# rafaelgmv/Distributed-Autonomous-Exploration-and-Mapping

Measured on AMD Instinct MI355X. Metric: beam-cell updates/sec + frontier-extract ms on 16384² grid, higher is better.
Workload: dtype int32/u32 ray math + fp32 log-odds (fp64 endpoints)

## Files before the change

distributed-autonomous-exploration-and-mapping_amd/csrc/dm_api.cpp:

```cpp
#include <math.h>
#include <stdarg.h>
#include <stdio.h>
#include <string.h>

#include <algorithm>
#include <new>
#include <string>
#include <vector>

#include "dm_internal.h"

#include <stdlib.h>

hipError_t dm_sync_all(dm_grid* g) {
  for (hipStream_t s : {g->stream, g->fe_stream, g->pass_stream, g->big_stream}) {
    if (!s) continue;
    const hipError_t e = hipStreamSynchronize(s);
    if (e != hipSuccess) return e;
  }
  g->p_pending = false;
  for (auto& f : g->fw) f.busy_pending = false;
  return hipSuccess;
}

// ... 452 lines not shown
  for (auto& w : g->iw) {
    if ((rc = dev_alloc(&w.tile_count, g->NT, "tile counts"))) return fail(rc);
    if ((rc = dev_alloc(&w.tile_cur, g->NT, "tile bin cursors"))) return fail(rc);
    if ((rc = dev_alloc(&w.cnt, CNT_N, "integrate counters"))) return fail(rc);
    if ((rc = dev_alloc(&w.sh, kShards * kShardWords, "integrate shard counters"))) return fail(rc);
    DM_HIP(hipMemset(w.cnt, 0, sizeof(unsigned long long) * CNT_N));
    DM_HIP(hipMemset(w.sh, 0, sizeof(unsigned long long) * kShards * kShardWords));
  }
  if ((rc = dev_alloc(&g->tile_free, g->NT, "tile free counts"))) return fail(rc);
  if ((rc = dev_alloc(&g->fmask, g->NT * DM_TILE * 16, "tile free / unknown bit rows"))) return fail(rc);
  if ((rc = dev_alloc(&g->fedge, g->NT * 4, "tile unknown edge words"))) return fail(rc);
  if ((rc = dev_alloc(&g->tile_seen, g->NT, "tile seen flags"))) return fail(rc);
  if (const char* sp = getenv("DM_SPARSE_PIECES")) g->sparse_pieces = std::max(0, atoi(sp));
  const char* fm = getenv("DM_FMASK");
  g->fmask_mode = fm && !strcmp(fm, "on") ? 1 : (fm && !strcmp(fm, "off") ? 2 : 0);
  const char* fk = getenv("DM_FRONTIER_KERNEL");
  g->frontier_kernel = fk && !strcmp(fk, "wave") ? 1 : (fk && !strcmp(fk, "wg") ? 2 : 0);
  if (const char* sm = getenv("DM_SORT_MIN")) g->sort_min = std::max<int64_t>(0, atoll(sm));
  g->fault_gate = dm_env_on("DM_FAULT_GATE");
  if (const char* pr = getenv("DM_PLAN_MAX_ROUNDS")) g->plan_max_rounds = std::max<int64_t>(0, atoll(pr));
  for (auto& f : g->fw) {
    e = hipEventCreateWithFlags(&f.ev_split, hipEventDisableTiming | hipEventDisableSystemFence);
    if (e != hipSuccess) return fail(dm_hip_check(e, "hipEventCreate"));
    if ((rc = dev_alloc(&f.cnt, CNT_N, "frontier counters"))) return fail(rc);
    DM_HIP(hipMemset(f.cnt, 0, sizeof(unsigned long long) * CNT_N));
    if ((rc = dev_alloc(&f.fsh, kShards * kShardWords, "frontier shard counters"))) return fail(rc);
    DM_HIP(hipMemset(f.fsh, 0, sizeof(unsigned long long) * kShards * kShardWords));
    if ((rc = dev_alloc(&f.big_tiles, g->NT, "frontier big tiles"))) return fail(rc);
    if ((rc = dev_alloc(&f.fbits, g->NT * DM_TILE, "frontier bit rows"))) return fail(rc);
    if ((rc = dev_alloc(&f.edge_slot, 2 * g->W, "edge slots"))) return fail(rc);
// ... 77 lines not shown
    if (ev) (void)hipEventDestroy(ev);
  for (auto& r : g->rb) {
    if (r.ev) (void)hipEventDestroy(r.ev);
    if (r.out_clu) (void)hipFree(r.out_clu - kRbRecords);
    if (r.h_out) (void)hipHostFree(r.h_out - kRbHostRecords);
    dev_free(r.m_out);
  }
  if (g->fe_stream) (void)hipStreamDestroy(g->fe_stream);
  if (g->pass_stream) (void)hipStreamDestroy(g->pass_stream);
  if (g->big_stream) (void)hipStreamDestroy(g->big_stream);
  for (auto& f : g->fw) {
    if (f.ev_split) (void)hipEventDestroy(f.ev_split);
    dev_free(f.cnt); dev_free(f.fsh); dev_free(f.big_tiles); dev_free(f.fbits);
    dev_free(f.edge_slot); dev_free(f.slot_parent);
  }
  dev_free(g->fl_n); dev_free(g->bits_flag);
  for (int i = 0; i < 2; ++i) { dev_free(g->flist[i]); dev_free(g->flist_n[i]); }
  for (int b = 0; b < 2; ++b) { dev_free(g->goal_k[b]); dev_free(g->goal_i[b]); }
  dev_free(g->goal_io); dev_free(g->goal_idx);
  dev_free(g->plan_cost); dev_free(g->plan_trav); dev_free(g->plan_travs); dev_free(g->plan_list[0]);
  dev_free(g->plan_list[1]); dev_free(g->plan_stamp); dev_free(g->plan_len); dev_free(g->plan_stat);
  dev_free(g->plan_src); dev_free(g->plan_qxy); dev_free(g->plan_qcost); dev_free(g->plan_qcell);
  dev_free(g->plan_path);
  if (g->h_plan) (void)hipHostFree(g->h_plan);
  dev_free(g->match_V); dev_free(g->match_kern); dev_free(g->match_tiles); dev_free(g->match_pose4);
  dev_free(g->match_trig); dev_free(g->match_ranges); dev_free(g->match_q); dev_free(g->match_vol);
  dev_free(g->match_out);
  dev_free(g->gain_xy); dev_free(g->gain_cell); dev_free(g->gain_out); dev_free(g->gain_skip);
  dev_free(g->gain_memo_cell); dev_free(g->gain_memo_gain);
  for (auto& w : g->iw) {
    dev_free(w.pieces); dev_free(w.hitems); dev_free(w.litems); dev_free(w.heavy_list); dev_free(w.slabs);
// ... 164 lines not shown
  const unsigned long long* fs = g->h_sh + kShards * kShardWords;
  const unsigned long long* ic = g->h_cnt + CNT_N;
  const uint64_t items = ic[CNT_ITEMS] + ic[CNT_LITEMS] + ic[CNT_SITEMS];
  const uint64_t pieces = ic[CNT_SEGS];
  const uint64_t v[kNStats] = {dm_shard_sum(g->h_sh, SH_U),  dm_shard_sum(g->h_sh, SH_T),
                               dm_shard_sum(g->h_sh, SH_TH), pieces,
                               ic[CNT_ACTIVE],               items,
                               ic[CNT_HEAVY],                g->h_cnt[CNT_FL0],
                               dm_shard_sum(fs, SH_SLOT),    g->h_cnt[CNT_CLUSTERS],
                               ic[CNT_SITEMS]};
  for (int32_t i = 0; i < cap && i < kNStats; ++i) out[i] = v[i];
  if (n_out) *n_out = kNStats;
  return DM_OK;
}

int dm_get_state(dm_grid* g, int8_t* out) {
  if (g && g->sh) return (out ? dm_sh_get_state(g, out) : dm_set_error(DM_ERR_INVALID_ARG, "out is NULL"));
  int rc = check_grid(g);
  if (rc || (rc = use_device(g))) return rc;
  if (!out) return dm_set_error(DM_ERR_INVALID_ARG, "out is NULL");
  DM_HIP(hipMemcpyAsync(out, g->state, (size_t)(g->W * g->R), hipMemcpyDeviceToHost, g->stream));
  DM_HIP(hipStreamSynchronize(g->stream));
  return DM_OK;
}

int dm_get_logodds(dm_grid* g, float* out) {
  if (g && g->sh) return (out ? dm_sh_get_logodds(g, out) : dm_set_error(DM_ERR_INVALID_ARG, "out is NULL"));
  int rc = check_grid(g);
  if (rc || (rc = use_device(g))) return rc;
  if (!out) return dm_set_error(DM_ERR_INVALID_ARG, "out is NULL");
// ... 85 lines not shown

int dm_frontiers_export_device(dm_grid* g, void* d_export, int64_t rec_cap) {
  if (int rc0 = not_on_sharded(g, "dm_frontiers_export_device")) return rc0;
  int rc = check_grid(g);
  if (rc || (rc = use_device(g))) return rc;
  if (!d_export || rec_cap < 0) return dm_set_error(DM_ERR_INVALID_ARG, "d_export is NULL or rec_cap < 0");
  if (g->p.min_frontier_size > 1)
    return dm_set_error(DM_ERR_INVALID_ARG,
                        "export needs a band handle with min_frontier_size <= 1 (the size filter "
                        "applies to merged clusters)");
  dm_select_slot(g, g->rb_count < dm_grid::kRbSlots ? (g->rb_head + g->rb_count) % dm_grid::kRbSlots
                                                    : dm_grid::kRbSync);
  hipStream_t es = g->stream;
  if ((rc = dm_enqueue_frontiers(g, false, false, g->overlap, &es))) return rc;
  if ((rc = dm_launch_export(g, es, d_export, rec_cap))) return rc;
  if (es != g->stream) {
    dm_grid::FrWs& f = g->fw[g->fparity];
    DM_HIP(hipEventRecord(f.ev_split, es));
    f.busy = f.ev_split;
    f.busy_pending = true;
    f.busy_pass = g->fr_pass;
    g->p_tail = f.ev_split;
    g->p_pending = true;
    g->p_tail_pass = g->fr_pass;
  } else {
    DM_HIP(dm_mark_ws_free(g));
  }
  g->frontier_valid = true;
  return DM_OK;
}
// ... 1097 lines not shown
```

distributed-autonomous-exploration-and-mapping_amd/csrc/dm_frontier.hip:

```cpp
#include "dm_internal.h"
#include "dm_uf.h"
#include "dm_phase.h"

#include <string.h>

#include <algorithm>

DM_PH_DECL(frontier)
DM_PH_DECL(ftile)

namespace {

constexpr int kFT = 256;
#ifndef DM_FT_OCC
#define DM_FT_OCC 7
#endif
constexpr int kMaxRoots = 1024;

struct FGeom {
  int32_t W, R, row0, TX, TY;
  int32_t has_before, has_after;
  int32_t pad_ = 0;
  int64_t NT;
  int32_t want_mask, want_labels;
// ... 18 lines not shown
__device__ inline void lds_unite(int32_t* par, int32_t a, int32_t b) {
  volatile int32_t* vp = par;
  for (int it = 0; it < 8192; ++it) {
    a = lds_find(vp, a);
    b = lds_find(vp, b);
    if (a == b) return;
    if (a < b) { const int32_t t = a; a = b; b = t; }
    const int32_t old = atomicMin(&par[a], b);
    if (old == a) return;
    a = old;
  }
}

constexpr int kMaxRuns = 2048;

__device__ inline uint64_t upto_mask(int p) {
  return p >= 63 ? ~0ull : ((2ull << p) - 1ull);
}

__device__ inline uint64_t run_starts(uint64_t F) { return F & ~(F << 1); }

__device__ inline int run_end(uint64_t F, int s0) {
  const uint64_t rest = ~(F >> s0);
  return rest ? s0 + __ffsll((unsigned long long)rest) - 2 : 63;
}

__device__ inline int run_of(const int32_t* rbase, const uint64_t* rowF, int y, int p) {
  return rbase[y] + __popcll(run_starts(rowF[y]) & upto_mask(p)) - 1;
}

__device__ inline int root_rank(const uint64_t* s_root, const int32_t* pre, int r) {
  return pre[r >> 6] + __popcll(s_root[r >> 6] & ((1ull << (r & 63)) - 1ull));
}

template <bool EDGE>
__global__ __launch_bounds__(kFT, DM_FT_OCC) void k_frontier_tile_big(
    FGeom g, const uint64_t* __restrict__ fbits, const int32_t* __restrict__ bflag,
    const int32_t* __restrict__ ftiles, const unsigned long long* __restrict__ list_n,
    int32_t* border, unsigned long long* rel,
    long long* __restrict__ slot_label, int32_t* slot_parent,
    long long* __restrict__ slot_own, long long* __restrict__ slot_acc,
    uint8_t* __restrict__ mask, int32_t* __restrict__ cell_slot, int32_t* __restrict__ edge_slot,
    unsigned long long* cnt, unsigned long long* fsh, int count_stats) {
  const unsigned long long stamp = cnt[CNT_STAMP];
  __shared__ uint64_t s_F[DM_TS];
  __shared__ int32_t s_rbase[DM_TS + 1];
  __shared__ int32_t r_par[kMaxRuns];
  __shared__ uint8_t r_s[kMaxRuns], r_y[kMaxRuns];
  __shared__ uint64_t s_root[kMaxRuns / 64];
  __shared__ int32_t s_rootpre[kMaxRuns / 64];
  __shared__ uint32_t szx[kMaxRoots], ssy[kMaxRoots];
  __shared__ int32_t nroots;
  __shared__ long long sbase;
  const int tid = threadIdx.x, lane = __lane_id();
  const int64_t nft = (int64_t)*list_n;
  const int64_t G = gridDim.x;
  __shared__ uint64_t s_todo;
  DM_PH_INIT();
  for (int64_t kb = blockIdx.x; kb < nft; kb += bflag ? 64 * G : G) {
  uint64_t todo = 1ull;
  if (bflag) {
    if (tid < 64) {
      const int64_t q = kb + (int64_t)tid * G;
      const uint64_t m = __ballot(q < nft && bflag[q] != 0);
      if (tid == 0) s_todo = m;
    }
    __syncthreads();
    todo = s_todo;
    __syncthreads();
  }
  while (todo) {
    const int64_t jj = bflag ? kb + (int64_t)(__ffsll((unsigned long long)todo) - 1) * G : kb;
    todo &= todo - 1;
    const int32_t tile = ftiles[jj];
    const uint64_t F = tid < DM_TS ? fbits[jj * DM_TS + tid] : 0ull;
    const int64_t j = tile;
    DM_PH_COUNT(dm_phase_acc_frontier, 16, 1);
    const int32_t tx0 = (tile % g.TX) * DM_TS;
    const int32_t ty0 = (tile / g.TX) * DM_TS;
    DM_PH(dm_phase_acc_frontier, 0);
    int any = 0;
    if (tid < DM_TS) {
      const int y = tid;
      const uint64_t st = run_starts(F);
      s_F[y] = F;
      any = F != 0ull;
      const int c = __popcll(st);
      int incl = c;
      for (int d = 1; d < 64; d <<= 1) {
        const int v = __shfl_up(incl, d);
        if (lane >= d) incl += v;
      }
      s_rbase[y] = incl - c;
      if (y == 63) s_rbase[DM_TS] = incl;
    }
    any = __syncthreads_or(any);
    DM_PH(dm_phase_acc_frontier, 1);
    if (!any) {
      __syncthreads();
      DM_PH(dm_phase_acc_frontier, 8);
      continue;
    }
    {
      const int y = tid >> 2, q = tid & 3;
      const uint64_t st_all = run_starts(s_F[y]);
      const uint64_t below = q ? upto_mask(16 * q - 1) : 0ull;
      uint64_t st = st_all & upto_mask(16 * q + 15) & ~below;
      int r = s_rbase[y] + __popcll(st_all & below);
      while (st) {
        const int s0 = __ffsll((unsigned long long)st) - 1;
        r_s[r] = (uint8_t)s0;
        r_y[r] = (uint8_t)y;
        r_par[r] = r;
        ++r;
        st &= st - 1;
      }
    }
    for (int r = tid; r < kMaxRoots; r += kFT) { szx[r] = 0; ssy[r] = 0; }
    __syncthreads();
    const int nruns = s_rbase[DM_TS];
    if (count_stats && tid == 0) {
      atomicAdd(&fsh[(blockIdx.x % kShards) * kShardWords + SH_RUNS], (unsigned long long)nruns);
      atomicAdd(&fsh[(blockIdx.x % kShards) * kShardWords + SH_FTF], 1ull);
    }
    DM_PH(dm_phase_acc_frontier, 2);
    DM_PH_COUNT(dm_phase_acc_frontier, 17, nruns);
    DM_PH_COUNT(dm_phase_acc_frontier, 18, 1);
    for (int r = tid; r < nruns; r += kFT) {
      const int y = r_y[r];
      if (y == 0) continue;
      const int s0 = r_s[r], e0 = run_end(s_F[y], s0);
      const int lo = s0 > 0 ? s0 - 1 : 0;
      const int hi = e0 < 63 ? e0 + 1 : 63;
      const uint64_t M = upto_mask(hi) & ~(lo > 0 ? upto_mask(lo - 1) : 0ull);
      uint64_t P = s_F[y - 1] & M;
      while (P) {
        const int p = __ffsll((unsigned long long)P) - 1;
        lds_unite(r_par, r, run_of(s_rbase, s_F, y - 1, p));
// ... 17 lines not shown
    __syncthreads();
    DM_PH(dm_phase_acc_frontier, 4);
    if (tid < 64) {
      const int nw = (nruns + 63) >> 6;
      const int c = tid < nw ? __popcll(s_root[tid]) : 0;
      int incl = c;
      for (int d = 1; d < 64; d <<= 1) {
        const int v = __shfl_up(incl, d);
        if (lane >= d) incl += v;
      }
      if (tid < nw) s_rootpre[tid] = incl - c;
      if (tid == 63) nroots = incl;
    }
    __syncthreads();
    DM_PH(dm_phase_acc_frontier, 5);
    if (tid == 0)
      sbase = (long long)atomicAdd(&fsh[(blockIdx.x % kShards) * kShardWords + SH_SLOT],
                                   (unsigned long long)nroots);
    for (int r = tid; r < nruns; r += kFT) {
      const int c = root_rank(s_root, s_rootpre, r_par[r]);
      const int y = r_y[r];
      const uint32_t s0 = r_s[r], e0 = (uint32_t)run_end(s_F[y], (int)s0), len = e0 - s0 + 1;
      atomicAdd(&szx[c], (len << 18) + (s0 + e0) * len / 2);
      atomicAdd(&ssy[c], (uint32_t)y * len);
    }
    __syncthreads();
    DM_PH(dm_phase_acc_frontier, 6);
    const long long base = sbase;
    const long long sh0 = (long long)(blockIdx.x % kShards) * g.slot_per;
    for (int r = tid; r < nruns; r += kFT) {
      if (r_par[r] != r) continue;
      const int c = root_rank(s_root, s_rootpre, r);
      if (base + c >= g.slot_per) { atomicOr(&cnt[CNT_OVERFLOW], kOvSlots); continue; }
      const long long slot = sh0 + base + c;
      const long long gy = (long long)g.row0 + ty0 + r_y[r];
      const long long gx = (long long)tx0 + r_s[r];
      const uint32_t zx = szx[c];
      const long long sz = zx >> 18;
      slot_label[slot] = gy * g.W + gx;
      const long long sx = sz * tx0 + (zx & 0x3FFFFu);
      const long long sy = sz * ((long long)g.row0 + ty0) + ssy[c];
      slot_own[3 * slot + 0] = sz; slot_own[3 * slot + 1] = sx; slot_own[3 * slot + 2] = sy;
      slot_acc[3 * slot + 0] = sz; slot_acc[3 * slot + 1] = sx; slot_acc[3 * slot + 2] = sy;
    }
    {
      const int side = tid >> 6, pos = lane;
      const int y = side == 0 ? 0 : side == 1 ? 63 : pos;
      const int x = side == 0 || side == 1 ? pos : side == 2 ? 0 : 63;
      int32_t sl = -1;
      if ((s_F[y] >> x) & 1ull) {
        const long long v = base + root_rank(s_root, s_rootpre, r_par[run_of(s_rbase, s_F, y, x)]);
        sl = v < g.slot_per ? (int32_t)(sh0 + v) : -1;
      }
      const uint64_t fb = __ballot(sl >= 0);
      if constexpr (EDGE) {
      if (fb) {
        border[j * 256 + tid] = sl;
        if (lane == 0) rel[4 * g.NT + 4 * j + side] = stamp;
      }
      } else {
      if (fb) {
        __hip_atomic_store(&border[j * 256 + tid], sl, __ATOMIC_RELAXED, __HIP_MEMORY_SCOPE_AGENT);
        asm volatile("s_waitcnt vmcnt(0)" ::: "memory");
        const int32_t tx = tile % g.TX, ty = tile / g.TX;
        const bool up = ty > 0, down = ty + 1 < g.TY, left = tx > 0, right = tx + 1 < g.TX;
        int64_t e = -1;
// ... 44 lines not shown
        }
        {
          const int32_t c0 = __shfl(sl, 0), c63 = __shfl(sl, 63);
          if (second && lane != 0) {
            const int32_t me = lane == 1 ? c0 : c63;
            const int nrow = side == 0 ? 1 : 0;
            const int ncol = lane == 1 ? 63 : 0;
            const int32_t b = __hip_atomic_load(&border[(int64_t)nb * 256 + nrow * 64 + ncol], __ATOMIC_RELAXED,
                                                __HIP_MEMORY_SCOPE_AGENT);
            if (me >= 0 && b >= 0) dm_uf_unite_idx(slot_parent, me, b, &cnt[CNT_OVERFLOW], kOvUnionFind);
          }
        }
      }
      }
    }
    const bool dense = g.want_mask || g.want_labels;
    if (dense || ty0 == 0 || ty0 + DM_TS >= g.R) {
      for (int c = tid; c < DM_TS * DM_TS; c += kFT) {
        const int y = c >> 6, x = c & 63;
        const int32_t gy = ty0 + y, gx = tx0 + x;
        if (gx >= g.W || gy >= g.R) continue;
        const bool edge = gy == 0 || gy == g.R - 1;
        if (!dense && !edge) continue;
        const bool f = (s_F[y] >> x) & 1ull;
        long long sl = -1;
        if (f) {
          sl = base + root_rank(s_root, s_rootpre, r_par[run_of(s_rbase, s_F, y, x)]);
          sl = sl < g.slot_per ? sh0 + sl : -1;
        }
        const int64_t gi = (int64_t)gy * g.W + gx;
        if (g.want_mask) mask[gi] = f;
        if (g.want_labels) cell_slot[gi] = (int32_t)sl;
        if (f) {
          if (gy == 0) edge_slot[gx] = (int32_t)sl;
          if (gy == g.R - 1) edge_slot[g.W + gx] = (int32_t)sl;
        }
      }
    }
    __syncthreads();
    DM_PH(dm_phase_acc_frontier, 7);
  }
  }
  DM_PH_FLUSH(dm_phase_acc_frontier);
}

constexpr int kFW = 4;
constexpr int64_t kDenseRuns = 48;
constexpr int64_t kDenseMaxTiles = 4096;
#ifndef DM_FL_RUNS
#define DM_FL_RUNS 384
#endif
constexpr int kRunsFast = DM_FL_RUNS;
#ifndef DM_FL_OCC
#define DM_FL_OCC 7
#endif
// ... 681 lines not shown
    clusters[4 * k + 2] = slot_acc[3 * s + 1];
    clusters[4 * k + 3] = slot_acc[3 * s + 2];
  }
}

__device__ inline void write_rb_header(int64_t K, int64_t cap, unsigned long long* sorted,
                                       const unsigned long long* __restrict__ cnt, int ncnt,
                                       int sorted_idx, const unsigned long long* __restrict__ fsh,
                                       dm_raw_record* host_out) {
  const int tid = threadIdx.x;
  if (tid == 0) *sorted = K <= cap ? 1ull : 0ull;
  if (!host_out) return;
  unsigned long long* header = dm_rb_header(host_out);
  if (tid < ncnt) header[tid] = tid == sorted_idx ? (K <= cap ? 1ull : 0ull) : cnt[tid];
  if (tid == ncnt && fsh) {
    unsigned long long most = 0, runs = 0, ftf = 0, big = 0;
    for (int i = 0; i < kShards; ++i) {
      most = max(most, fsh[i * kShardWords + SH_SLOT]);
      runs += fsh[i * kShardWords + SH_RUNS];
      ftf += fsh[i * kShardWords + SH_FTF];
      big += fsh[i * kShardWords + SH_BIG];
    }
    header[ncnt] = most;
    header[ncnt + 1] = runs;
    header[ncnt + 2] = ftf;
    header[ncnt + 3] = big;
  }
}

__device__ inline void record_vals(const long long* clusters, const long long* sums, const long long* labels,
                                   int64_t i, long long* lab, long long* sz, long long* sx, long long* sy) {
  const long long m = clusters[4 * i + 1];
  if (sums && m < 0) {
    const int64_t sl = -m - 1;
    *lab = labels[sl];
    *sz = sums[3 * sl];
    *sx = sums[3 * sl + 1];
    *sy = sums[3 * sl + 2];
  } else {
    *lab = clusters[4 * i];
    *sz = m;
// ... 383 lines not shown
  const bool want_off = g->fmask_mode == 2 || (g->fmask_mode == 0 && g->ftile_hint < kFmaskOnTiles / 4);
  if (!g->fmask_on && want_on) {
    if (!g->fmask_valid) {
      if (int rc = dm_launch_recount(g)) return rc;
    }
    g->fmask_on = true;
  } else if (g->fmask_on && want_off) {
    g->fmask_on = false;
  }
  const bool dense = g->frontier_kernel == 2 ||
                     (g->frontier_kernel == 0 && g->ftf_hint > 0 && g->runs_hint > kDenseRuns * g->ftf_hint &&
                      g->ftf_hint <= kDenseMaxTiles);
  const bool edge = !dense && g->sort_hint <= std::max<int64_t>(g->ftile_hint, 1);
  auto* const big_kernel = edge ? k_frontier_tile_big<true> : k_frontier_tile_big<false>;
  auto* const wave_kernel = edge ? k_frontier_tile<true> : k_frontier_tile<false>;
  dm_timer_begin(g, "frontier_bits", &t);
  DM_LAUNCH(k_frontier_bits, dim3(bits_grid), dim3(kFW * 64), 0, g->stream, fg, g->state, g->halo, g->fmask,
            g->fedge, g->tile_seen, g->ftiles, g->ftiles_n, list_n, g->fbits, g->cnt, g->fmask_on ? 1 : 0,
            dense ? nullptr : g->big_tiles, g->fsh, g->edge_slot, 2 * g->W, g->slot_parent, g->fe_flag + kHaltWord,
            g->bits_flag + kStampWord);
  dm_timer_end(g, &t);
  DM_HIP(hipGetLastError());
  hipStream_t ps = g->stream;
  if (split) {
    ps = g->pass_stream;
    hipEvent_t eb = g->ev_bits[g->fparity];
    DM_HIP(hipEventRecord(eb, g->stream));
    DM_HIP(dm_mark_ws_free(g, eb));
    DM_HIP(hipStreamWaitEvent(ps, eb, 0));
  }
  if (end_stream) *end_stream = ps;
  if (!dense) {
    const int big_grid =
        grid_for(std::min<int64_t>(g->NT, dm_quantize_up(g->big_hint + g->big_hint / 4 + 64)), 1, 8192);
    DM_HIP(hipEventRecord(g->ev_bigfork, ps));
    DM_HIP(hipStreamWaitEvent(g->big_stream, g->ev_bigfork, 0));
    dm_timer_begin(g, "frontier_big", &t, g->big_stream);
    DM_LAUNCH(big_kernel, dim3(big_grid), dim3(kFT), 0, g->big_stream, fg, g->fbits,
              g->big_tiles,
              g->ftiles, list_n, g->border, g->rel, g->slot_label, g->slot_parent, g->slot_own,
              g->slot_acc, g->mask, g->cell_slot, g->edge_slot, g->cnt, g->fsh, 0);
    dm_timer_end(g, &t);
    DM_HIP(hipGetLastError());
    DM_HIP(hipEventRecord(g->ev_big, g->big_stream));
    dm_timer_begin(g, "frontier_tile", &t, ps);
    DM_LAUNCH(wave_kernel, dim3(wave_grid), dim3(kFW * 64), 0, ps, fg, g->fbits,
                       g->ftiles, list_n, g->border, g->rel,
                       g->slot_label, g->slot_parent, g->slot_own, g->slot_acc, g->mask, g->cell_slot,
                       g->edge_slot, g->cnt, g->fsh, g->big_tiles);
    dm_timer_end(g, &t);
    DM_HIP(hipGetLastError());
    DM_HIP(hipStreamWaitEvent(ps, g->ev_big, 0));
  } else {
    dm_timer_begin(g, "frontier_tile", &t, ps);
    const int dense_grid = grid_for(std::min<int64_t>(g->NT, g->ftile_hint > 0 ? want_waves : g->NT), 1, 8192);
    DM_LAUNCH(big_kernel, dim3(dense_grid), dim3(kFT), 0, ps, fg, g->fbits, nullptr,
              g->ftiles, list_n,
              g->border, g->rel, g->slot_label, g->slot_parent, g->slot_own, g->slot_acc, g->mask,
              g->cell_slot, g->edge_slot, g->cnt, g->fsh, 1);
    dm_timer_end(g, &t);
    DM_HIP(hipGetLastError());
  }
  if (edge) {
    dm_timer_begin(g, "frontier_edges", &t, ps);
    DM_LAUNCH(k_frontier_edges, dim3(grid_for(std::min<int64_t>(want_waves, g->NT), kFW, 16384)),
              dim3(kFW * 64), 0, ps, fg, g->ftiles, list_n, g->border, g->rel,
              g->slot_parent, g->cnt);
    dm_timer_end(g, &t);
    DM_HIP(hipGetLastError());
  }
  const int sgrid = grid_for(g->slot_cap, 256, 1024);
  dm_timer_begin(g, "frontier_resolve", &t, ps);
  const int fuse = g->p.min_frontier_size <= 1 ? 1 : 0;
  DM_LAUNCH(k_frontier_resolve, dim3(grid_for(g->slot_cap, 256, g->n_cu)), dim3(256), 0, ps, fg,
// ... 36 lines not shown
    return dm_set_error(DM_ERR_PIPELINE, "the overlapped pipeline's front-end hand-off timed out: a map "
                                         "update was skipped; dm_reset the handle");
  if ((int64_t)most > g->slot_cap / kShards || (g->h_cnt[CNT_OVERFLOW] & kOvSlots)) {
    *n_clusters = (int64_t)most * kShards;
    return DM_ERR_CAPACITY;
  }
  if (g->h_cnt[CNT_OVERFLOW] & kOvUnionFind)
    return dm_set_error(DM_ERR_INCOMPLETE, "frontier union-find did not converge within its bound "
                                           "(dm_uf.h): this pass has no result");
  *n_clusters = (int64_t)g->h_cnt[CNT_CLUSTERS];
  g->sort_hint = *n_clusters;
  g->ftile_hint = (int64_t)g->h_cnt[CNT_FL0];
  g->runs_hint = (int64_t)hdr[CNT_N + 1];
  g->ftf_hint = (int64_t)hdr[CNT_N + 2];
  g->big_hint = (int64_t)hdr[CNT_N + 3];
  return DM_OK;
}

int dm_launch_frontiers(dm_grid* g, bool want_mask, bool want_labels, int64_t* n_clusters,
                        int64_t* copied) {
  int rc = dm_enqueue_frontiers(g, want_mask, want_labels);
  if (rc) return rc;
  DM_HIP(hipStreamSynchronize(g->stream));
  return dm_frontiers_readback(g, n_clusters, copied);
}
```

distributed-autonomous-exploration-and-mapping_amd/csrc/dm_internal.h:

```cpp
#pragma once

#include <hip/hip_runtime.h>
#include <stdint.h>

#include <atomic>
#include <chrono>
#include <string>
#include <vector>

#include "../../include/dm.h"

#include "dm_ray.h"


enum {
  CNT_ACTIVE = 0,
  CNT_U = 1,
  CNT_T = 2,
  CNT_SEGS = 3,
  CNT_FTILES = 4,
  CNT_SLOTS = 5,
  CNT_CLUSTERS = 6,
  CNT_OVERFLOW = 7,
  CNT_ITEMS = 8,
// ... 14 lines not shown
constexpr int kHaltWord = 8;
constexpr int kSigWord = 0;
constexpr int kGateWord = 4;
constexpr int kStampWord = 8;
constexpr int kIntegrateCounters[] = {CNT_ACTIVE, CNT_U, CNT_T, CNT_SEGS, CNT_ITEMS,
                                      CNT_HEAVY, CNT_TH, CNT_LITEMS, CNT_IOVERFLOW, CNT_SITEMS};

constexpr int kIntegrateChunk = 256;
constexpr int kIntegrateMedium = 1024;


constexpr int kShards = 32;
constexpr int kShardWords = 16;
static_assert(kShards * kShardWords == 512, "k_integrate_reset covers 512 shard words");
enum { SH_U = 0, SH_T = 1, SH_TH = 2, SH_ACT = 3 };
enum { SH_SLOT = 0, SH_RUNS = 1, SH_FTF = 2, SH_BIG = 3 };

constexpr int kNStats = 11;
constexpr bool dm_stat_is_frontier(int i) { return i >= 7 && i <= 9; }

constexpr int kRbRecords = 6;
static_assert(kRbRecords * sizeof(dm_cluster) >= (CNT_N + 4) * sizeof(unsigned long long), "readback header");
struct dm_raw_record {
  long long label, size, sum_x, sum_y;
};
constexpr int kRbHostRecords = 6;
static_assert(kRbHostRecords * sizeof(dm_raw_record) >= (CNT_N + 4) * sizeof(unsigned long long),
              "readback header");
__host__ __device__ inline unsigned long long* dm_rb_header(dm_raw_record* records) {
  return reinterpret_cast<unsigned long long*>(records - kRbHostRecords);
}
__host__ __device__ inline const unsigned long long* dm_rb_header(const dm_raw_record* records) {
  return reinterpret_cast<const unsigned long long*>(records - kRbHostRecords);
}
__host__ __device__ inline double dm_centroid(double origin, long long sum, long long size, double res) {
  const double m = (double)sum / (double)size;
  return origin + (m + 0.5) * res;
}

struct dm_grid;
hipError_t dm_copy_shards(dm_grid* g);
inline unsigned long long dm_shard_sum(const unsigned long long* sh, int field) {
// ... 48 lines not shown
  int cur_slot = 0;
  uint64_t rb_gen = 0;
  uint64_t fr_pass = 0, m_pass = 0;
  int64_t W = 0, H = 0, R = 0, row0 = 0;
  int64_t TX = 0, TY = 0, NT = 0;
  int32_t nmax = 0;

  float* L = nullptr;
  int8_t* state = nullptr;
  int32_t* tile_free = nullptr;
  uint8_t* fmask = nullptr;
  uint64_t* fedge = nullptr;
  uint8_t* tile_seen = nullptr;
  bool fmask_on = false, fmask_valid = false;
  int fmask_mode = 0;
  unsigned long long* cnt = nullptr;
  unsigned long long* h_cnt = nullptr;
  unsigned long long* fsh = nullptr;
  unsigned long long* h_sh = nullptr;

  int64_t beams_cap = 0;
  int64_t blk_cap = 0;
  int64_t segs_cap = 0;
  int64_t act_cap = 0;
  int64_t hitem_cap = 0;
  int64_t heavy_cap = 0;
  struct IntWs {
    Beam* beams = nullptr;
    int2* blk_hist = nullptr;
    int32_t* blk_n = nullptr;
// ... 310 lines not shown
int dm_match_launch_scans(dm_grid* g, int32_t S, int32_t N, int32_t A, int32_t k0, int32_t sub, int32_t half,
                          int32_t stride);
int dm_launch_ld06(dm_grid* g, int32_t S, const dm_ld06_point* d_pts, const int64_t* d_offsets,
                   int32_t N, int dir, float* d_ranges, float* d_intensities);

int dm_sh_destroy(dm_grid* g);
int dm_sh_reset(dm_grid* g);
int dm_sh_integrate(dm_grid* g, int32_t S, const double* poses, int32_t N, const float* ranges, float amin,
                    float inc, uint64_t* U, uint64_t* T);
int dm_sh_integrate_async(dm_grid* g, int32_t S, const double* poses, int32_t N, const float* ranges,
                          float amin, float inc);
int dm_sh_integrate_device(dm_grid* g, int32_t S, const double* d_pose4, int32_t N, const float* d_ranges,
                           float amin, float inc);
int dm_sh_last_counts(dm_grid* g, uint64_t* U, uint64_t* T);
int dm_sh_last_stats(dm_grid* g, uint64_t* out, int32_t cap, int32_t* n_out);
int dm_sh_get_state(dm_grid* g, int8_t* out);
int dm_sh_get_logodds(dm_grid* g, float* out);
int dm_sh_set_logodds(dm_grid* g, const float* in);
int dm_sh_set_state(dm_grid* g, const int8_t* in);
int dm_sh_frontiers(dm_grid* g, uint8_t* mask, int64_t* labels, dm_cluster* out, int64_t cap, int64_t* n_out);
int dm_sh_frontiers_begin(dm_grid* g);
int dm_sh_frontiers_end(dm_grid* g, dm_cluster* out, int64_t cap, int64_t* n_out);
int dm_sh_frontiers_poll(dm_grid* g, int32_t* ready);
int dm_sh_assign_goals(dm_grid* g, const double* robots_xy, int32_t n_robots, int64_t min_size, double w,
                       double min_distance, int64_t* out_index, double* out_xy);
int dm_sh_set_overlap(dm_grid* g, int32_t on);
int dm_sh_synchronize(dm_grid* g);
int dm_sh_profile_enable(dm_grid* g, int enable);
int dm_sh_profile_read(dm_grid* g, dm_kernel_stat* out, int32_t cap, int32_t* n_out);
int dm_sh_profile_reset(dm_grid* g);
// ... 28 lines not shown
```

distributed-autonomous-exploration-and-mapping_amd/csrc/dm_sharded.cpp:

```cpp
#include <string.h>

#include <algorithm>
#include <new>
#include <numeric>
#include <vector>

#include "dm_internal.h"

namespace {

constexpr int kSets = 2;

struct Staging {
  double* poses = nullptr;
  float* ranges = nullptr;
  int64_t pose_cap = 0, ranges_cap = 0;
};

int64_t ceil_div(int64_t a, int64_t b) { return (a + b - 1) / b; }

template <class T>
int dev_alloc_on(int dev, T** p, int64_t count, const char* what) {
  (void)hipSetDevice(dev);
  if (*p) { (void)hipFree(*p); *p = nullptr; }
// ... 480 lines not shown
  dm_shard_set* s = g->sh;
  if (cap > 0 && !out) return dm_set_error(DM_ERR_INVALID_ARG, "out is NULL");
  uint64_t sum[kNStats] = {0};
  for (int r = 0; r < s->P; ++r) {
    uint64_t v[kNStats] = {0};
    int32_t n = 0;
    if (int rc = dm_last_stats(s->band[(size_t)r], v, kNStats, &n)) return rc;
    for (int i = 0; i < kNStats; ++i)
      if (s->active[(size_t)r] || dm_stat_is_frontier(i)) sum[i] += v[i];
  }
  for (int32_t i = 0; i < cap && i < kNStats; ++i) out[i] = sum[i];
  if (n_out) *n_out = kNStats;
  return DM_OK;
}

int dm_sh_profile_enable(dm_grid* g, int enable) {
  dm_shard_set* s = g->sh;
  for (int r = 0; r < s->P; ++r)
    if (int rc = dm_profile_enable(s->band[(size_t)r], enable)) return rc;
  return DM_OK;
}

int dm_sh_profile_read(dm_grid* g, dm_kernel_stat* out, int32_t cap, int32_t* n_out) {
  dm_shard_set* s = g->sh;
  std::vector<dm_kernel_stat> all;
  for (int r = 0; r < s->P; ++r) {
    int32_t n = 0;
    if (int rc = dm_profile_read(s->band[(size_t)r], nullptr, 0, &n)) return rc;
    std::vector<dm_kernel_stat> v((size_t)std::max(n, 1));
    if (int rc = dm_profile_read(s->band[(size_t)r], v.data(), n, &n)) return rc;
// ... 187 lines not shown
```

distributed-autonomous-exploration-and-mapping_amd/dm/_ffi.py:

```python
from __future__ import annotations

import ctypes
import os
import threading

_HERE = os.path.dirname(os.path.abspath(__file__))
LIB_PATH = os.environ.get("DM_LIB", os.path.join(_HERE, "libdm.so"))

DM_OK = 0
DM_ERR_INVALID_ARG = -1
DM_ERR_SHAPE = -2
DM_ERR_HIP = -3
DM_ERR_OOM = -4
DM_ERR_CAPACITY = -5
DM_ERR_IO = -6
DM_ERR_STATE = -7
DM_ERR_INCOMPLETE = -8
DM_ERR_PIPELINE = -9
DM_ERR_COLLECTIVE = -10
DM_TILE = 64
DM_PLAN_UNREACHABLE = 0xFFFFFFFF

_ERR_NAMES = {
    DM_ERR_INVALID_ARG: "DM_ERR_INVALID_ARG",
# ... 90 lines not shown

SIGNATURES = {
    "dm_default_params": [ctypes.POINTER(DmParams), _i64, _i64],
    "dm_create": [ctypes.POINTER(_vp), ctypes.POINTER(DmParams), ctypes.c_int],
    "dm_create_sharded": [ctypes.POINTER(_vp), ctypes.POINTER(DmParams), _i32, ctypes.POINTER(_i32)],
    "dm_sharded_band_rows": [_i64, _i32, _i32, ctypes.POINTER(_i64), ctypes.POINTER(_i64)],
    "dm_sharded_info": [_vp, ctypes.POINTER(_i32), ctypes.POINTER(_i64)],
    "dm_destroy": [_vp],
    "dm_reset": [_vp],
    "dm_get_params": [_vp, ctypes.POINTER(DmParams)],
    "dm_integrate": [_vp, _i32, _vp, _i32, _vp, _f32, _f32, _vp, _vp],
    "dm_integrate_device": [_vp, _i32, _vp, _i32, _vp, _f32, _f32],
    "dm_integrate_async": [_vp, _i32, _vp, _i32, _vp, _f32, _f32],
    "dm_last_counts": [_vp, _vp, _vp],
    "dm_last_stats": [_vp, _vp, _i32, ctypes.POINTER(_i32)],
    "dm_get_state": [_vp, _vp],
    "dm_get_logodds": [_vp, _vp],
    "dm_set_logodds": [_vp, _vp],
    "dm_set_state": [_vp, _vp],
    "dm_frontiers": [_vp, _vp, _vp, _vp, _i64, ctypes.POINTER(_i64)],
    "dm_set_halo": [_vp, _vp, _vp],
    "dm_set_halo_device": [_vp, _vp, _vp],
    "dm_get_edge_rows": [_vp, _vp, _vp],
    "dm_get_edge_rows_device": [_vp, _vp, _vp],
    "dm_get_edge_labels": [_vp, _vp, _vp],
    "dm_save": [_vp, ctypes.c_char_p],
    "dm_load": [_vp, ctypes.c_char_p],
    "dm_set_stream": [_vp, _vp],
    "dm_exchange_stream": [_vp, ctypes.POINTER(ctypes.c_void_p)],
    "dm_synchronize": [_vp],
# ... 80 lines not shown
```

distributed-autonomous-exploration-and-mapping_amd/dm/grid.py:

```python
from __future__ import annotations

import ctypes
import threading
from dataclasses import dataclass

import numpy as np

from . import _ffi
from ._ffi import CLUSTER_DTYPE, DmError, DmParams, check, load_library


def default_params(width: int, height: int, **overrides) -> DmParams:
    lib = load_library()
    p = DmParams()
    check(lib.dm_default_params(ctypes.byref(p), int(width), int(height)))
    res_given = "resolution" in overrides
    for k, v in overrides.items():
        if not hasattr(p, k):
            raise DmError(_ffi.DM_ERR_INVALID_ARG, f"unknown parameter {k!r}")
        setattr(p, k, v)
    if res_given and "origin_x" not in overrides:
        p.origin_x = -0.5 * p.width * p.resolution
    if res_given and "origin_y" not in overrides:
        p.origin_y = -0.5 * p.height * p.resolution
# ... 117 lines not shown
        with self._lock:
            check(self._lib.dm_last_counts(self._handle(), ctypes.byref(U), ctypes.byref(T)))
        return int(U.value), int(T.value)

    STAT_NAMES = ("updates", "touched", "touched_heavy", "pieces", "active_tiles", "work_items",
                  "heavy_tiles", "frontier_tiles", "frontier_slots", "frontier_clusters", "sparse_items")

    def last_stats(self) -> dict:
        k = len(self.STAT_NAMES)
        out = (ctypes.c_uint64 * k)()
        n = ctypes.c_int32(0)
        with self._lock:
            check(self._lib.dm_last_stats(self._handle(), out, k, ctypes.byref(n)))
        return {k: int(out[i]) for i, k in enumerate(self.STAT_NAMES)}

    def ld06_to_scans(self, points, offsets, n_beams: int, laser_scan_dir: bool = True,
                      want_intensities: bool = False):
        pts = np.ascontiguousarray(points, dtype=np.dtype(_ffi.LD06_POINT_DTYPE))
        off = np.ascontiguousarray(offsets, dtype=np.int64)
        S = off.shape[0] - 1
        ranges = np.empty((S, n_beams), np.float32)
        inten = np.empty((S, n_beams), np.float32) if want_intensities else None
        with self._lock:
            check(self._lib.dm_ld06_to_scans(self._handle(), S, _vp(pts), _vp(off), int(n_beams),
                                             1 if laser_scan_dir else 0, _vp(ranges), _vp(inten)))
        return (ranges, inten) if want_intensities else ranges

    def state(self) -> np.ndarray:
        out = np.empty((self.rows, self.width), np.int8)
        with self._lock:
# ... 358 lines not shown
```

include/dm.h:

```cpp
#ifndef DM_H
#define DM_H

#include <stddef.h>
#include <stdint.h>

#ifdef __cplusplus
extern "C" {
#endif

#define DM_OK 0
#define DM_ERR_INVALID_ARG (-1)
#define DM_ERR_SHAPE (-2)
#define DM_ERR_HIP (-3)
#define DM_ERR_OOM (-4)
#define DM_ERR_CAPACITY (-5)
#define DM_ERR_IO (-6)
#define DM_ERR_STATE (-7)
#define DM_ERR_INCOMPLETE (-8)
#define DM_ERR_PIPELINE (-9)
#define DM_ERR_COLLECTIVE (-10)

#define DM_TILE 64

#define DM_PLAN_UNREACHABLE 0xFFFFFFFFu
// ... 42 lines not shown
int dm_get_params(const dm_grid* g, dm_params* out);

int dm_integrate(dm_grid* g, int32_t S, const double* poses, int32_t N,
                 const float* ranges, float angle_min, float angle_increment,
                 uint64_t* out_updates, uint64_t* out_touched);

int dm_integrate_async(dm_grid* g, int32_t S, const double* poses, int32_t N,
                       const float* ranges, float angle_min, float angle_increment);

int dm_integrate_device(dm_grid* g, int32_t S, const double* d_pose4,
                        int32_t N, const float* d_ranges, float angle_min,
                        float angle_increment);
int dm_last_counts(dm_grid* g, uint64_t* updates, uint64_t* touched);

int dm_last_stats(dm_grid* g, uint64_t* out, int32_t cap, int32_t* n_out);

int dm_get_state(dm_grid* g, int8_t* out);
int dm_get_logodds(dm_grid* g, float* out);
int dm_set_logodds(dm_grid* g, const float* in);
int dm_set_state(dm_grid* g, const int8_t* in);

int dm_frontiers(dm_grid* g, uint8_t* mask, int64_t* labels, dm_cluster* out,
                 int64_t cap, int64_t* n_out);

int dm_frontiers_begin(dm_grid* g);
int dm_frontiers_end(dm_grid* g, dm_cluster* out, int64_t cap, int64_t* n_out);
int dm_frontiers_poll(dm_grid* g, int32_t* ready);
int dm_max_passes_in_flight(void);

int dm_set_overlap(dm_grid* g, int32_t on);
// ... 90 lines not shown
```

Measured before the change: 211.2 billion.

## Cache per-tile frontier labeling keyed on tile bit pattern across calls

Adds a per-tile device cache that stores each frontier tile's bit rows, component summaries and edge ranks. When a tile's frontier bits match the cached entry (and no dense output is needed), the kernel skips run union-find and root ranking and emits slots directly from the cached component records. This removes the union-find work for tiles that are unchanged between extractions. It costs extra memory (160 words per tile), an extra cache read and compare on every tile, and cache writes on misses.

```diff
diff --git a/distributed-autonomous-exploration-and-mapping_amd/csrc/dm_api.cpp b/distributed-autonomous-exploration-and-mapping_amd/csrc/dm_api.cpp
--- a/distributed-autonomous-exploration-and-mapping_amd/csrc/dm_api.cpp
+++ b/distributed-autonomous-exploration-and-mapping_amd/csrc/dm_api.cpp
@@ -490,6 +490,8 @@
   if (const char* sp = getenv("DM_SPARSE_PIECES")) g->sparse_pieces = std::max(0, atoi(sp));
   const char* fm = getenv("DM_FMASK");
   g->fmask_mode = fm && !strcmp(fm, "on") ? 1 : (fm && !strcmp(fm, "off") ? 2 : 0);
+  const char* fc = getenv("DM_FRONTIER_CACHE");
+  g->fcache_mode = fc && !strcmp(fc, "off") ? 0 : 1;
   const char* fk = getenv("DM_FRONTIER_KERNEL");
   g->frontier_kernel = fk && !strcmp(fk, "wave") ? 1 : (fk && !strcmp(fk, "wg") ? 2 : 0);
   if (const char* sm = getenv("DM_SORT_MIN")) g->sort_min = std::max<int64_t>(0, atoll(sm));
@@ -597,7 +599,7 @@
     dev_free(f.cnt); dev_free(f.fsh); dev_free(f.big_tiles); dev_free(f.fbits);
     dev_free(f.edge_slot); dev_free(f.slot_parent);
   }
-  dev_free(g->fl_n); dev_free(g->bits_flag);
+  dev_free(g->fl_n); dev_free(g->bits_flag); dev_free(g->fcache);
   for (int i = 0; i < 2; ++i) { dev_free(g->flist[i]); dev_free(g->flist_n[i]); }
   for (int b = 0; b < 2; ++b) { dev_free(g->goal_k[b]); dev_free(g->goal_i[b]); }
   dev_free(g->goal_io); dev_free(g->goal_idx);
@@ -792,6 +794,24 @@
   return DM_OK;
 }
 
+int dm_frontier_cache_stats(dm_grid* g, uint64_t* hits, uint64_t* misses) {
+  if (g && g->sh) return dm_sh_frontier_cache_stats(g, hits, misses);
+  int rc = check_grid(g);
+  if (rc || (rc = use_device(g))) return rc;
+  if (!hits || !misses) return dm_set_error(DM_ERR_INVALID_ARG, "hits or misses is NULL");
+  if (!g->fc_collected) {
+    DM_HIP(dm_sync_all(g));
+    DM_HIP(hipMemcpy(g->h_sh + kShards * kShardWords, g->fsh, sizeof(unsigned long long) * kShards * kShardWords,
+                     hipMemcpyDeviceToHost));
+    g->fc_hits = dm_shard_sum(g->h_sh + kShards * kShardWords, SH_CHIT);
+    g->fc_misses = dm_shard_sum(g->h_sh + kShards * kShardWords, SH_CMISS);
+    g->fc_collected = true;
+  }
+  *hits = g->fc_hits;
+  *misses = g->fc_misses;
+  return DM_OK;
+}
+
 int dm_get_state(dm_grid* g, int8_t* out) {
   if (g && g->sh) return (out ? dm_sh_get_state(g, out) : dm_set_error(DM_ERR_INVALID_ARG, "out is NULL"));
   int rc = check_grid(g);
@@ -907,6 +927,7 @@
   hipStream_t es = g->stream;
   if ((rc = dm_enqueue_frontiers(g, false, false, g->overlap, &es))) return rc;
   if ((rc = dm_launch_export(g, es, d_export, rec_cap))) return rc;
+  g->fc_collected = false;
   if (es != g->stream) {
     dm_grid::FrWs& f = g->fw[g->fparity];
     DM_HIP(hipEventRecord(f.ev_split, es));
diff --git a/distributed-autonomous-exploration-and-mapping_amd/csrc/dm_frontier.hip b/distributed-autonomous-exploration-and-mapping_amd/csrc/dm_frontier.hip
--- a/distributed-autonomous-exploration-and-mapping_amd/csrc/dm_frontier.hip
+++ b/distributed-autonomous-exploration-and-mapping_amd/csrc/dm_frontier.hip
@@ -56,6 +56,10 @@
 
 constexpr int kMaxRuns = 2048;
 
+constexpr int kCacheRoots = 62;
+constexpr int kFcHdr = 64, kFcEdge = 65, kFcComp = 97;
+static_assert(kFcComp + kCacheRoots <= kFcWords && kCacheRoots < 0xFF, "label cache entry layout");
+
 __device__ inline uint64_t upto_mask(int p) {
   return p >= 63 ? ~0ull : ((2ull << p) - 1ull);
 }
@@ -83,7 +87,7 @@
     long long* __restrict__ slot_label, int32_t* slot_parent,
     long long* __restrict__ slot_own, long long* __restrict__ slot_acc,
     uint8_t* __restrict__ mask, int32_t* __restrict__ cell_slot, int32_t* __restrict__ edge_slot,
-    unsigned long long* cnt, unsigned long long* fsh, int count_stats) {
+    unsigned long long* cnt, unsigned long long* fsh, int count_stats, uint64_t* fcache) {
   const unsigned long long stamp = cnt[CNT_STAMP];
   __shared__ uint64_t s_F[DM_TS];
   __shared__ int32_t s_rbase[DM_TS + 1];
@@ -94,10 +98,11 @@
   __shared__ uint32_t szx[kMaxRoots], ssy[kMaxRoots];
   __shared__ int32_t nroots;
   __shared__ long long sbase;
-  const int tid = threadIdx.x, lane = __lane_id();
+  int tid = threadIdx.x;
   const int64_t nft = (int64_t)*list_n;
   const int64_t G = gridDim.x;
   __shared__ uint64_t s_todo;
+  __shared__ uint32_t s_match;
   DM_PH_INIT();
   for (int64_t kb = blockIdx.x; kb < nft; kb += bflag ? 64 * G : G) {
   uint64_t todo = 1ull;
@@ -114,12 +119,22 @@
   while (todo) {
     const int64_t jj = bflag ? kb + (int64_t)(__ffsll((unsigned long long)todo) - 1) * G : kb;
     todo &= todo - 1;
+    asm volatile("" : "+v"(tid));
+    const int lane = tid & 63;
     const int32_t tile = ftiles[jj];
     const uint64_t F = tid < DM_TS ? fbits[jj * DM_TS + tid] : 0ull;
     const int64_t j = tile;
     DM_PH_COUNT(dm_phase_acc_frontier, 16, 1);
     const int32_t tx0 = (tile % g.TX) * DM_TS;
     const int32_t ty0 = (tile / g.TX) * DM_TS;
+    const bool dense = g.want_mask || g.want_labels;
+    const bool band_edge = ty0 == 0 || ty0 + DM_TS >= g.R;
+    uint64_t* const ent = fcache && !band_edge ? fcache + (int64_t)tile * kFcWords : nullptr;
+    uint64_t c_hdr = 0, c_F = 0;
+    if (ent && tid < DM_TS) {
+      c_hdr = ent[kFcHdr];
+      c_F = ent[tid];
+    }
     DM_PH(dm_phase_acc_frontier, 0);
     int any = 0;
     if (tid < DM_TS) {
@@ -135,14 +150,57 @@
       }
       s_rbase[y] = incl - c;
       if (y == 63) s_rbase[DM_TS] = incl;
+      const uint64_t same = __ballot(c_F == F);
+      if (y == 0) s_match = (c_hdr & 1ull) && same == ~0ull ? (uint32_t)c_hdr : 0u;
     }
     any = __syncthreads_or(any);
+    const uint32_t c_info = s_match;
+    const bool match = c_info != 0u;
+    const bool hit = match && !dense;
     DM_PH(dm_phase_acc_frontier, 1);
     if (!any) {
       __syncthreads();
       DM_PH(dm_phase_acc_frontier, 8);
       continue;
     }
+    long long base = 0;
+    uint32_t c_edge = 0xFFu;
+    const long long sh0 = (long long)(blockIdx.x % kShards) * g.slot_per;
+    unsigned long long* const shard = fsh + (blockIdx.x % kShards) * kShardWords;
+    if (hit) {
+    const int nr = (int)((c_info >> 8) & 0xFFu);
+    const uint64_t c_comp = tid < nr ? ent[kFcComp + tid] : 0ull;
+    c_edge = reinterpret_cast<const uint8_t*>(ent + kFcEdge)[tid];
+    if (tid == 0) {
+      sbase = (long long)atomicAdd(&shard[SH_SLOT], (unsigned long long)nr);
+      if (count_stats) {
+        atomicAdd(&shard[SH_RUNS], (unsigned long long)(c_info >> 16));
+        atomicAdd(&shard[SH_FTF], 1ull);
+      }
+      atomicAdd(&shard[SH_CHIT], 1ull);
+    }
+    __syncthreads();
+    DM_PH(dm_phase_acc_frontier, 9);
+    DM_PH_COUNT(dm_phase_acc_frontier, 18, 1);
+    DM_PH_COUNT(dm_phase_acc_frontier, 19, 1);
+    base = sbase;
+    if (tid < nr) {
+      if (base + tid >= g.slot_per) {
+        atomicOr(&cnt[CNT_OVERFLOW], kOvSlots);
+      } else {
+        const long long slot = sh0 + base + tid;
+        const long long gy = (long long)g.row0 + ty0 + (long long)((c_comp >> 6) & 63u);
+        const long long gx = (long long)tx0 + (long long)(c_comp & 63u);
+        const long long sz = (long long)((c_comp >> 12) & 0x1FFFu);
+        slot_label[slot] = gy * g.W + gx;
+        const long long sx = sz * tx0 + (long long)((c_comp >> 25) & 0x3FFFFu);
+        const long long sy = sz * ((long long)g.row0 + ty0) + (long long)((c_comp >> 43) & 0x3FFFFu);
+        slot_own[3 * slot + 0] = sz; slot_own[3 * slot + 1] = sx; slot_own[3 * slot + 2] = sy;
+        slot_acc[3 * slot + 0] = sz; slot_acc[3 * slot + 1] = sx; slot_acc[3 * slot + 2] = sy;
+      }
+    }
+    DM_PH(dm_phase_acc_frontier, 10);
+    } else {
     {
       const int y = tid >> 2, q = tid & 3;
       const uint64_t st_all = run_starts(s_F[y]);
@@ -161,9 +219,12 @@
     for (int r = tid; r < kMaxRoots; r += kFT) { szx[r] = 0; ssy[r] = 0; }
     __syncthreads();
     const int nruns = s_rbase[DM_TS];
-    if (count_stats && tid == 0) {
-      atomicAdd(&fsh[(blockIdx.x % kShards) * kShardWords + SH_RUNS], (unsigned long long)nruns);
-      atomicAdd(&fsh[(blockIdx.x % kShards) * kShardWords + SH_FTF], 1ull);
+    if (tid == 0) {
+      if (count_stats) {
+        atomicAdd(&shard[SH_RUNS], (unsigned long long)nruns);
+        atomicAdd(&shard[SH_FTF], 1ull);
+      }
+      if (fcache) atomicAdd(&shard[SH_CMISS], 1ull);
     }
     DM_PH(dm_phase_acc_frontier, 2);
     DM_PH_COUNT(dm_phase_acc_frontier, 17, nruns);
@@ -211,9 +272,7 @@
     }
     __syncthreads();
     DM_PH(dm_phase_acc_frontier, 5);
-    if (tid == 0)
-      sbase = (long long)atomicAdd(&fsh[(blockIdx.x % kShards) * kShardWords + SH_SLOT],
-                                   (unsigned long long)nroots);
+    if (tid == 0) sbase = (long long)atomicAdd(&shard[SH_SLOT], (unsigned long long)nroots);
     for (int r = tid; r < nruns; r += kFT) {
       const int c = root_rank(s_root, s_rootpre, r_par[r]);
       const int y = r_y[r];
@@ -223,8 +282,7 @@
     }
     __syncthreads();
     DM_PH(dm_phase_acc_frontier, 6);
-    const long long base = sbase;
-    const long long sh0 = (long long)(blockIdx.x % kShards) * g.slot_per;
+    base = sbase;
     for (int r = tid; r < nruns; r += kFT) {
       if (r_par[r] != r) continue;
       const int c = root_rank(s_root, s_rootpre, r);
@@ -240,13 +298,20 @@
       slot_own[3 * slot + 0] = sz; slot_own[3 * slot + 1] = sx; slot_own[3 * slot + 2] = sy;
       slot_acc[3 * slot + 0] = sz; slot_acc[3 * slot + 1] = sx; slot_acc[3 * slot + 2] = sy;
     }
+    }
     {
       const int side = tid >> 6, pos = lane;
       const int y = side == 0 ? 0 : side == 1 ? 63 : pos;
       const int x = side == 0 || side == 1 ? pos : side == 2 ? 0 : 63;
       int32_t sl = -1;
-      if ((s_F[y] >> x) & 1ull) {
-        const long long v = base + root_rank(s_root, s_rootpre, r_par[run_of(s_rbase, s_F, y, x)]);
+      int crank = -1;
+      if (hit) {
+        if (c_edge != 0xFFu) crank = (int)c_edge;
+      } else if ((s_F[y] >> x) & 1ull) {
+        crank = root_rank(s_root, s_rootpre, r_par[run_of(s_rbase, s_F, y, x)]);
+      }
+      if (crank >= 0) {
+        const long long v = base + crank;
         sl = v < g.slot_per ? (int32_t)(sh0 + v) : -1;
       }
       const uint64_t fb = __ballot(sl >= 0);
@@ -321,8 +386,7 @@
       }
       }
     }
-    const bool dense = g.want_mask || g.want_labels;
-    if (dense || ty0 == 0 || ty0 + DM_TS >= g.R) {
+    if (dense || band_edge) {
       for (int c = tid; c < DM_TS * DM_TS; c += kFT) {
         const int y = c >> 6, x = c & 63;
         const int32_t gy = ty0 + y, gx = tx0 + x;
@@ -344,8 +408,39 @@
         }
       }
     }
-    __syncthreads();
-    DM_PH(dm_phase_acc_frontier, 7);
+    if (ent && !match) {
+#ifdef DM_PHASE_TIMING
+      __syncthreads();
+      DM_PH(dm_phase_acc_frontier, 7);
+#endif
+      const int nr = nroots, nruns = s_rbase[DM_TS];
+      if (nr > kCacheRoots) {
+        if (tid == 0) ent[kFcHdr] = 0ull;
+      } else {
+        if (tid < DM_TS) ent[tid] = s_F[tid];
+        {
+          const int side = tid >> 6;
+          const int y = side == 0 ? 0 : side == 1 ? 63 : lane;
+          const int x = side == 0 || side == 1 ? lane : side == 2 ? 0 : 63;
+          uint8_t rk = 0xFFu;
+          if ((s_F[y] >> x) & 1ull) rk = (uint8_t)root_rank(s_root, s_rootpre, r_par[run_of(s_rbase, s_F, y, x)]);
+          reinterpret_cast<uint8_t*>(ent + kFcEdge)[tid] = rk;
+        }
+        for (int r = tid; r < nruns; r += kFT) {
+          if (r_par[r] != r) continue;
+          const int c = root_rank(s_root, s_rootpre, r);
+          const uint64_t zx = szx[c];
+          ent[kFcComp + c] = (uint64_t)r_s[r] | ((uint64_t)r_y[r] << 6) | ((zx >> 18) << 12) |
+                             ((zx & 0x3FFFFull) << 25) | ((uint64_t)ssy[c] << 43);
+        }
+        if (tid == 0) ent[kFcHdr] = 1ull | ((uint64_t)nr << 8) | ((uint64_t)nruns << 16);
+      }
+      __syncthreads();
+      DM_PH(dm_phase_acc_frontier, 11);
+    } else {
+      __syncthreads();
+      DM_PH(dm_phase_acc_frontier, 7);
+    }
   }
   }
   DM_PH_FLUSH(dm_phase_acc_frontier);
@@ -1057,17 +1152,21 @@
   unsigned long long* header = dm_rb_header(host_out);
   if (tid < ncnt) header[tid] = tid == sorted_idx ? (K <= cap ? 1ull : 0ull) : cnt[tid];
   if (tid == ncnt && fsh) {
-    unsigned long long most = 0, runs = 0, ftf = 0, big = 0;
+    unsigned long long most = 0, runs = 0, ftf = 0, big = 0, chit = 0, cmiss = 0;
     for (int i = 0; i < kShards; ++i) {
       most = max(most, fsh[i * kShardWords + SH_SLOT]);
       runs += fsh[i * kShardWords + SH_RUNS];
       ftf += fsh[i * kShardWords + SH_FTF];
       big += fsh[i * kShardWords + SH_BIG];
+      chit += fsh[i * kShardWords + SH_CHIT];
+      cmiss += fsh[i * kShardWords + SH_CMISS];
     }
     header[ncnt] = most;
     header[ncnt + 1] = runs;
     header[ncnt + 2] = ftf;
     header[ncnt + 3] = big;
+    header[ncnt + 4] = chit;
+    header[ncnt + 5] = cmiss;
   }
 }
 
@@ -1481,6 +1580,17 @@
   const bool edge = !dense && g->sort_hint <= std::max<int64_t>(g->ftile_hint, 1);
   auto* const big_kernel = edge ? k_frontier_tile_big<true> : k_frontier_tile_big<false>;
   auto* const wave_kernel = edge ? k_frontier_tile<true> : k_frontier_tile<false>;
+  if (g->fcache_mode == 1 && !g->fcache) {
+    void* p = nullptr;
+    const size_t bytes = sizeof(uint64_t) * kFcWords * (size_t)g->NT;
+    if (hipMalloc(&p, bytes) == hipSuccess && hipMemsetAsync(p, 0, bytes, g->stream) == hipSuccess) {
+      g->fcache = (uint64_t*)p;
+    } else {
+      (void)hipGetLastError();
+      if (p) (void)hipFree(p);
+      g->fcache_mode = 0;
+    }
+  }
   dm_timer_begin(g, "frontier_bits", &t);
   DM_LAUNCH(k_frontier_bits, dim3(bits_grid), dim3(kFW * 64), 0, g->stream, fg, g->state, g->halo, g->fmask,
             g->fedge, g->tile_seen, g->ftiles, g->ftiles_n, list_n, g->fbits, g->cnt, g->fmask_on ? 1 : 0,
@@ -1506,7 +1616,7 @@
     DM_LAUNCH(big_kernel, dim3(big_grid), dim3(kFT), 0, g->big_stream, fg, g->fbits,
               g->big_tiles,
               g->ftiles, list_n, g->border, g->rel, g->slot_label, g->slot_parent, g->slot_own,
-              g->slot_acc, g->mask, g->cell_slot, g->edge_slot, g->cnt, g->fsh, 0);
+              g->slot_acc, g->mask, g->cell_slot, g->edge_slot, g->cnt, g->fsh, 0, g->fcache);
     dm_timer_end(g, &t);
     DM_HIP(hipGetLastError());
     DM_HIP(hipEventRecord(g->ev_big, g->big_stream));
@@ -1524,7 +1634,7 @@
     DM_LAUNCH(big_kernel, dim3(dense_grid), dim3(kFT), 0, ps, fg, g->fbits, nullptr,
               g->ftiles, list_n,
               g->border, g->rel, g->slot_label, g->slot_parent, g->slot_own, g->slot_acc, g->mask,
-              g->cell_slot, g->edge_slot, g->cnt, g->fsh, 1);
+              g->cell_slot, g->edge_slot, g->cnt, g->fsh, 1, g->fcache);
     dm_timer_end(g, &t);
     DM_HIP(hipGetLastError());
   }
@@ -1591,6 +1701,9 @@
   g->runs_hint = (int64_t)hdr[CNT_N + 1];
   g->ftf_hint = (int64_t)hdr[CNT_N + 2];
   g->big_hint = (int64_t)hdr[CNT_N + 3];
+  g->fc_hits = hdr[CNT_N + 4];
+  g->fc_misses = hdr[CNT_N + 5];
+  g->fc_collected = true;
   return DM_OK;
 }
 
diff --git a/distributed-autonomous-exploration-and-mapping_amd/csrc/dm_internal.h b/distributed-autonomous-exploration-and-mapping_amd/csrc/dm_internal.h
--- a/distributed-autonomous-exploration-and-mapping_amd/csrc/dm_internal.h
+++ b/distributed-autonomous-exploration-and-mapping_amd/csrc/dm_internal.h
@@ -52,18 +52,19 @@
 constexpr int kShardWords = 16;
 static_assert(kShards * kShardWords == 512, "k_integrate_reset covers 512 shard words");
 enum { SH_U = 0, SH_T = 1, SH_TH = 2, SH_ACT = 3 };
-enum { SH_SLOT = 0, SH_RUNS = 1, SH_FTF = 2, SH_BIG = 3 };
+enum { SH_SLOT = 0, SH_RUNS = 1, SH_FTF = 2, SH_BIG = 3, SH_CHIT = 4, SH_CMISS = 5 };
+constexpr int kFcWords = 160;
 
 constexpr int kNStats = 11;
 constexpr bool dm_stat_is_frontier(int i) { return i >= 7 && i <= 9; }
 
 constexpr int kRbRecords = 6;
-static_assert(kRbRecords * sizeof(dm_cluster) >= (CNT_N + 4) * sizeof(unsigned long long), "readback header");
+static_assert(kRbRecords * sizeof(dm_cluster) >= (CNT_N + 6) * sizeof(unsigned long long), "readback header");
 struct dm_raw_record {
   long long label, size, sum_x, sum_y;
 };
 constexpr int kRbHostRecords = 6;
-static_assert(kRbHostRecords * sizeof(dm_raw_record) >= (CNT_N + 4) * sizeof(unsigned long long),
+static_assert(kRbHostRecords * sizeof(dm_raw_record) >= (CNT_N + 6) * sizeof(unsigned long long),
               "readback header");
 __host__ __device__ inline unsigned long long* dm_rb_header(dm_raw_record* records) {
   return reinterpret_cast<unsigned long long*>(records - kRbHostRecords);
@@ -142,6 +143,10 @@
   uint8_t* tile_seen = nullptr;
   bool fmask_on = false, fmask_valid = false;
   int fmask_mode = 0;
+  uint64_t* fcache = nullptr;
+  int fcache_mode = 1;
+  unsigned long long fc_hits = 0, fc_misses = 0;
+  bool fc_collected = true;
   unsigned long long* cnt = nullptr;
   unsigned long long* h_cnt = nullptr;
   unsigned long long* fsh = nullptr;
@@ -482,6 +487,7 @@
                            float amin, float inc);
 int dm_sh_last_counts(dm_grid* g, uint64_t* U, uint64_t* T);
 int dm_sh_last_stats(dm_grid* g, uint64_t* out, int32_t cap, int32_t* n_out);
+int dm_sh_frontier_cache_stats(dm_grid* g, uint64_t* hits, uint64_t* misses);
 int dm_sh_get_state(dm_grid* g, int8_t* out);
 int dm_sh_get_logodds(dm_grid* g, float* out);
 int dm_sh_set_logodds(dm_grid* g, const float* in);
diff --git a/distributed-autonomous-exploration-and-mapping_amd/csrc/dm_sharded.cpp b/distributed-autonomous-exploration-and-mapping_amd/csrc/dm_sharded.cpp
--- a/distributed-autonomous-exploration-and-mapping_amd/csrc/dm_sharded.cpp
+++ b/distributed-autonomous-exploration-and-mapping_amd/csrc/dm_sharded.cpp
@@ -518,6 +518,21 @@
   return DM_OK;
 }
 
+int dm_sh_frontier_cache_stats(dm_grid* g, uint64_t* hits, uint64_t* misses) {
+  dm_shard_set* s = g->sh;
+  if (!hits || !misses) return dm_set_error(DM_ERR_INVALID_ARG, "hits or misses is NULL");
+  uint64_t h = 0, m = 0;
+  for (int r = 0; r < s->P; ++r) {
+    uint64_t bh = 0, bm = 0;
+    if (int rc = dm_frontier_cache_stats(s->band[(size_t)r], &bh, &bm)) return rc;
+    h += bh;
+    m += bm;
+  }
+  *hits = h;
+  *misses = m;
+  return DM_OK;
+}
+
 int dm_sh_profile_enable(dm_grid* g, int enable) {
   dm_shard_set* s = g->sh;
   for (int r = 0; r < s->P; ++r)
diff --git a/distributed-autonomous-exploration-and-mapping_amd/dm/_ffi.py b/distributed-autonomous-exploration-and-mapping_amd/dm/_ffi.py
--- a/distributed-autonomous-exploration-and-mapping_amd/dm/_ffi.py
+++ b/distributed-autonomous-exploration-and-mapping_amd/dm/_ffi.py
@@ -128,6 +128,7 @@
     "dm_integrate_async": [_vp, _i32, _vp, _i32, _vp, _f32, _f32],
     "dm_last_counts": [_vp, _vp, _vp],
     "dm_last_stats": [_vp, _vp, _i32, ctypes.POINTER(_i32)],
+    "dm_frontier_cache_stats": [_vp, ctypes.POINTER(ctypes.c_uint64), ctypes.POINTER(ctypes.c_uint64)],
     "dm_get_state": [_vp, _vp],
     "dm_get_logodds": [_vp, _vp],
     "dm_set_logodds": [_vp, _vp],
diff --git a/distributed-autonomous-exploration-and-mapping_amd/dm/grid.py b/distributed-autonomous-exploration-and-mapping_amd/dm/grid.py
--- a/distributed-autonomous-exploration-and-mapping_amd/dm/grid.py
+++ b/distributed-autonomous-exploration-and-mapping_amd/dm/grid.py
@@ -155,6 +155,12 @@
             check(self._lib.dm_last_stats(self._handle(), out, k, ctypes.byref(n)))
         return {k: int(out[i]) for i, k in enumerate(self.STAT_NAMES)}
 
+    def frontier_cache_stats(self) -> tuple[int, int]:
+        h, m = ctypes.c_uint64(0), ctypes.c_uint64(0)
+        with self._lock:
+            check(self._lib.dm_frontier_cache_stats(self._handle(), ctypes.byref(h), ctypes.byref(m)))
+        return int(h.value), int(m.value)
+
     def ld06_to_scans(self, points, offsets, n_beams: int, laser_scan_dir: bool = True,
                       want_intensities: bool = False):
         pts = np.ascontiguousarray(points, dtype=np.dtype(_ffi.LD06_POINT_DTYPE))
diff --git a/include/dm.h b/include/dm.h
--- a/include/dm.h
+++ b/include/dm.h
@@ -80,6 +80,8 @@
 int dm_last_counts(dm_grid* g, uint64_t* updates, uint64_t* touched);
 
 int dm_last_stats(dm_grid* g, uint64_t* out, int32_t cap, int32_t* n_out);
+
+int dm_frontier_cache_stats(dm_grid* g, uint64_t* hits, uint64_t* misses);
 
 int dm_get_state(dm_grid* g, int8_t* out);
 int dm_get_logodds(dm_grid* g, float* out);
```

After: 222.7 billion (median of 6 runs). +5.4%, better.
